# Ren-Okubo/diffusion_model

Hardware: AMD Instinct MI355X
Metric: atoms*denoise-steps/sec, 64-atom SiO2 T=1000 (higher is better)
Workload: dtype bf16; 1 GPU; 64-atom SiO2 cells x 256 graphs/GPU, 4-layer EGNN (H=36, W=1024, m=256), T=1000 reverse steps, fully connected (E=1032192/GPU); global_batch=256, parallelism=replicas x1 (no data-path collective)

## Files before the change

diffusion_model_amd/csrc/edge_tile.h:

```cpp
#pragma once
#include "kernels.h"

namespace egnn {
namespace tile128 {

constexpr int kR = 128;
static_assert(kR == kTileRows, "plan_forward (host_logic.cpp) plans 128-edge tiles");
constexpr int kSegFast = 8;
constexpr int kTileThreads = 512;
constexpr int kChunkK = 64;
constexpr int kRowPad = kR + 1;
constexpr size_t kChunkBytes = (size_t)8 * kRowPad * 16;
constexpr size_t kStageBytes = (size_t)8 * 32 * 72 * 2;
constexpr size_t kOffDst = 0;
constexpr size_t kOffSrc = kOffDst + kR * 4;
constexpr size_t kOffD2 = kOffSrc + kR * 4;
constexpr size_t kOffDiff = kOffD2 + kR * 4;
constexpr size_t kOffVal = kOffDiff + 3 * kR * 4;
constexpr size_t kOffPart = kOffVal + kR * 4;
constexpr size_t kOffSegRow = kOffPart + 8 * kR * 4;
constexpr size_t kOffSegNode = kOffSegRow + kR * 4;
constexpr size_t kOffSegRs = kOffSegNode + kR * 4;
constexpr size_t kOffSegRe = kOffSegRs + kR * 4;
constexpr size_t kOffSegMode = kOffSegRe + kR * 4;
constexpr size_t kOffMisc = kOffSegMode + kR * 4;
constexpr size_t kOffGseg = kOffMisc + 64;
constexpr size_t kOffLoop = kOffGseg + kSegFast * kR * 4;

#define TILE_LDS_RD(dst, base, off) asm volatile("ds_read_b128 %0, %1 offset:%2" : "=v"(dst) : "v"(base), "n"(off))
#define TILE_LDS_WAIT(n) asm volatile("s_waitcnt lgkmcnt(" #n ")" ::: "memory")

struct Lds {
  int *dst, *src, *seg_of_row, *seg_node, *seg_rs, *seg_re, *seg_mode, *misc;
  float *d2, *diff, *val, *part, *gseg;
  __device__ __forceinline__ explicit Lds(char* smem)
      : dst(reinterpret_cast<int*>(smem + kOffDst)), src(reinterpret_cast<int*>(smem + kOffSrc)),
        seg_of_row(reinterpret_cast<int*>(smem + kOffSegRow)), seg_node(reinterpret_cast<int*>(smem + kOffSegNode)),
        seg_rs(reinterpret_cast<int*>(smem + kOffSegRs)), seg_re(reinterpret_cast<int*>(smem + kOffSegRe)),
        seg_mode(reinterpret_cast<int*>(smem + kOffSegMode)), misc(reinterpret_cast<int*>(smem + kOffMisc)),
        d2(reinterpret_cast<float*>(smem + kOffD2)), diff(reinterpret_cast<float*>(smem + kOffDiff)),
        val(reinterpret_cast<float*>(smem + kOffVal)), part(reinterpret_cast<float*>(smem + kOffPart)),
        gseg(reinterpret_cast<float*>(smem + kOffGseg)) {}
};

__device__ __forceinline__ void prologue_rows(const EdgeParams& p, const Lds& L, int e0, int nvalid, const float* wd, int KP,
                                              float* s_wd, int tid) {
  if (tid < kR) {
    int d = 0, s = 0;
    float dx = 0.f, dy = 0.f, dz = 0.f;
    if (tid < nvalid) {
      d = p.edge_dst[e0 + tid];
      s = p.edge_src[e0 + tid];
      dx = p.x[3 * d] - p.x[3 * s];
      dy = p.x[3 * d + 1] - p.x[3 * s + 1];
      dz = p.x[3 * d + 2] - p.x[3 * s + 2];
    }
    L.dst[tid] = d;
    L.src[tid] = s;
    L.diff[tid] = dx; L.diff[kR + tid] = dy; L.diff[2 * kR + tid] = dz;
    const float nrm = sqrtf(dx * dx + dy * dy + dz * dz);
    L.d2[tid] = nrm * nrm;
  }
  for (int i = tid; i < KP; i += 512) s_wd[i] = wd[i];
  __syncthreads();
}

__device__ __forceinline__ int segment_mode(const EdgeParams& p, const Lds& L, int e0, int seg) {
  const int n = L.seg_node[seg];
  const bool first = (e0 + L.seg_rs[seg]) == p.row_ptr[n];
  const bool last = (e0 + L.seg_re[seg] + 1) == p.row_ptr[n + 1];
  return (first && last) ? 2 : (first ? 1 : 0);
}

template <bool WITH_MODES = true>
__device__ __forceinline__ int prologue_segments(const EdgeParams& p, const Lds& L, int e0, int nvalid, int tid, int lane, int wave) {
  bool is_start = false, is_end = false;
  unsigned long long starts = 0;
  if (tid < kR) {
    const bool valid = tid < nvalid;
    const int d = L.dst[tid];
    is_start = valid && (tid == 0 || L.dst[tid - 1] != d);
    is_end = valid && (tid == nvalid - 1 || L.dst[tid + 1] != d);
    starts = __ballot(is_start);
    if (lane == 0) L.misc[1 + wave] = __popcll(starts);
  }
  __syncthreads();
  if (tid < kR) {
    const int seg = (wave == 1 ? L.misc[1] : 0) + __popcll(starts & ((2ull << lane) - 1ull)) - 1;
    L.seg_of_row[tid] = tid < nvalid ? seg : -1;
    if (is_start) { L.seg_node[seg] = L.dst[tid]; L.seg_rs[seg] = tid; }
    if (is_end) L.seg_re[seg] = tid;
    if (tid == 0) L.misc[0] = L.misc[1] + L.misc[2];
  }
  __syncthreads();
  const int S = L.misc[0];
  if constexpr (WITH_MODES) {
    if (tid < S) L.seg_mode[tid] = segment_mode(p, L, e0, tid);
  }
  return S;
}

__device__ __forceinline__ int prologue(const EdgeParams& p, const Lds& L, int e0, int nvalid, const float* wd, int KP,
                                        float* s_wd, int tid, int lane, int wave) {
  prologue_rows(p, L, e0, nvalid, wd, KP, s_wd, tid);
  return prologue_segments(p, L, e0, nvalid, tid, lane, wave);
}

template <int ESZ>
struct BuildRows {
  int brow, kg;
  unsigned vdst0, vsrc0, vdst1, vsrc1, offP, offQ;
  float d2r0, d2r1;
  rsrc_t tab;
  __device__ __forceinline__ unsigned row_off(const EdgeParams& p, int node) const {
    return (unsigned)node * (unsigned)p.TC * (unsigned)ESZ + (unsigned)kg * (8u * ESZ);
  }
  __device__ __forceinline__ BuildRows(const EdgeParams& p, const Lds& L, int tid, bool is_m, unsigned table_bytes, int d0, int s0,
                                       int d1, int s1)
      : brow(tid >> 3), kg(tid & 7), vdst0(row_off(p, d0)), vsrc0(row_off(p, s0)), vdst1(row_off(p, d1)), vsrc1(row_off(p, s1)),
        offP((is_m ? 2u * p.WxP : 0u) * ESZ), offQ((is_m ? 2u * p.WxP + p.WmP : (unsigned)p.WxP) * ESZ), d2r0(L.d2[brow]),
        d2r1(L.d2[brow + 64]), tab(make_rsrc(p.table, table_bytes)) {}
  __device__ __forceinline__ BuildRows(const EdgeParams& p, const Lds& L, int tid, bool is_m, unsigned table_bytes)
      : brow(tid >> 3), kg(tid & 7), vdst0(row_off(p, L.dst[brow])), vsrc0(row_off(p, L.src[brow])),
        vdst1(row_off(p, L.dst[brow + 64])), vsrc1(row_off(p, L.src[brow + 64])), offP((is_m ? 2u * p.WxP : 0u) * ESZ),
        offQ((is_m ? 2u * p.WxP + p.WmP : (unsigned)p.WxP) * ESZ), d2r0(L.d2[brow]), d2r1(L.d2[brow + 64]),
        tab(make_rsrc(p.table, table_bytes)) {}
};

template <class MPhase, class VFinish, class VLoad>
__device__ __forceinline__ void phase_opposed_k_loop(int NC, int wave, MPhase&& mphase, VFinish&& vfinish, VLoad&& vload) {
  if (wave < 4) {
    vload(1);
    for (int i = 0; i < NC - 1; ++i) {
      mphase(i, false);
      vfinish(i + 1);
      vload(i + 2);
      __syncthreads();
    }
    mphase(NC - 1, true);
    __syncthreads();
  } else {
    vload(1);
    for (int i = 0; i < NC - 1; ++i) {
      vfinish(i + 1);
      vload(i + 2);
      __builtin_amdgcn_sched_barrier(0);
      mphase(i, false);
      __syncthreads();
    }
    mphase(NC - 1, true);
    __syncthreads();
  }
}

template <int CB>
__device__ __forceinline__ void stage_store_rows(const f32x16 (&acc)[4][CB], char* stage, __bf16* out, size_t ld, int nvalid,
                                                 int lane, int wave) {
  static_assert(CB == 1 || CB == 2, "store_block_bf16 takes one or two 32-column blocks");
  __bf16* stg = reinterpret_cast<__bf16*>(stage) + (size_t)wave * 32 * 72;
#pragma unroll
  for (int rb = 0; rb < 4; ++rb) {
    f32x16 blk[2];
    blk[0] = acc[rb][0];
    blk[1] = acc[rb][CB - 1];
    store_block_bf16(blk, CB, stg, out + (size_t)(32 * rb) * ld, ld, nvalid - 32 * rb, lane);
  }
}

__device__ __forceinline__ void coordinate_segment_sums(const EdgeParams& p, const Lds& L, int S, int tile, int half, int tid,
                                                        int lane, int wave) {
  float* aggx = p.agg_x + (size_t)half * p.agg_x_stride;
  float* partx = p.part_x + (size_t)half * p.part_x_stride;
  if (S <= kSegFast) {
    if (wave < S) {
      const int seg = wave;
      float a0 = 0.f, a1 = 0.f, a2 = 0.f, a3 = 0.f;
#pragma unroll
      for (int u = 0; u < 2; ++u) {
        const int row = lane + 64 * u;
        if (L.seg_of_row[row] == seg) {
          const float sv = L.val[row];
          const float dx = L.diff[row], dy = L.diff[kR + row], dz = L.diff[2 * kR + row];
          a0 += dx * sv; a1 += dy * sv; a2 += dz * sv;
          a3 += dx * dx + dy * dy + dz * dz;
        }
      }
#pragma unroll
      for (int m = 32; m >= 1; m >>= 1) { a0 += __shfl_xor(a0, m); a1 += __shfl_xor(a1, m); a2 += __shfl_xor(a2, m); a3 += __shfl_xor(a3, m); }
      if (lane < 4) {
        const int mode = L.seg_mode[seg];
        float* dstp = mode == 2 ? aggx + (size_t)L.seg_node[seg] * 4 : partx + ((size_t)tile * 2 + mode) * 4;
        dstp[lane] = lane == 0 ? a0 : (lane == 1 ? a1 : (lane == 2 ? a2 : a3));
      }
    }
  } else {
    for (int t = tid; t < 4 * S; t += 512) {
      const int seg = t >> 2, d = t & 3, mode = L.seg_mode[seg];
      float sum = 0.f;
      if (d < 3) {
        for (int rr = L.seg_rs[seg]; rr <= L.seg_re[seg]; ++rr) sum += L.diff[d * kR + rr] * L.val[rr];
      } else {
        for (int rr = L.seg_rs[seg]; rr <= L.seg_re[seg]; ++rr) {
          const float dx = L.diff[rr], dy = L.diff[kR + rr], dz = L.diff[2 * kR + rr];
          sum += dx * dx + dy * dy + dz * dz;
        }
      }
      float* dstp = mode == 2 ? aggx + (size_t)L.seg_node[seg] * 4 : partx + ((size_t)tile * 2 + mode) * 4;
      dstp[d] = sum;
    }
  }
}



template <int CB, bool PRE_SCALED = false, bool STORE_SHARE = false>
__device__ __forceinline__ void x_head(const EdgeParams& p, const Lds& L, const f32x16 (&acc)[4][CB], int colblk0, int half,
                                       int tid, int lane, int wave, const float acc_scale = kNegLog2e, int e0 = 0,
                                       int nvalid = 0) {
  const int r = lane & 31;
  float part[64];
#pragma unroll
  for (int q = 0; q < 64; ++q) part[q] = 0.f;
#pragma unroll
  for (int cb = 0; cb < CB; ++cb) {
    const int n = 32 * (colblk0 + cb) + r;
    const float bb = p.b2x[n], w = p.w3x[n];
#pragma unroll
    for (int rb = 0; rb < 4; ++rb)
#pragma unroll
      for (int i = 0; i < 16; ++i)
        part[rb * 16 + i] = fmaf(w, silu_s(PRE_SCALED ? acc[rb][cb][i] : fmaf(acc[rb][cb][i], acc_scale, bb)), part[rb * 16 + i]);
  }
  {
    float lo[32], hi[32];
#pragma unroll
    for (int q = 0; q < 32; ++q) { lo[q] = part[q]; hi[q] = part[32 + q]; }
    const float t0 = butterfly32(lo, lane), t1 = butterfly32(hi, lane);
    const int row = 32 * (r >> 4) + acc_row(r & 15, lane);
    L.part[wave * kR + row] = t0;
    L.part[wave * kR + 64 + row] = t1;
  }
  __syncthreads();
  if (tid < kR) {
    float v = half == 0 ? p.scal[0] : 0.f;
#pragma unroll
    for (int w = 0; w < 8; ++w) v += L.part[w * kR + tid];
    L.val[tid] = v;
    if constexpr (STORE_SHARE) { if (tid < nvalid) p.s_half_out[(size_t)half * p.E + e0 + tid] = v; }
  }
  __syncthreads();
}

template <bool PRE_SCALED = false>
__device__ __forceinline__ void message_epilogue(const EdgeParams& p, const Lds& L, const f32x16 (&acc)[4][1], int S, int tile,
                                                 int tid, int lane, int wave, const float acc_scale = kNegLog2e,
                                                 const int colblk = -1) {
  const int r = lane & 31, hh = lane >> 5;
  const int ncol = 32 * (colblk < 0 ? wave : colblk) + r;
  float mval[64];
  {
    const float bb = p.b2m[ncol], wa = p.wa[ncol];
    float lo[32], hi[32];
#pragma unroll
    for (int rb = 0; rb < 4; ++rb)
#pragma unroll
      for (int i = 0; i < 16; ++i) {
        const float m = silu_s(PRE_SCALED ? acc[rb][0][i] : fmaf(acc[rb][0][i], acc_scale, bb));
        mval[rb * 16 + i] = m;
        if (rb < 2) lo[rb * 16 + i] = wa * m; else hi[(rb - 2) * 16 + i] = wa * m;
      }
    const float t0 = butterfly32(lo, lane), t1 = butterfly32(hi, lane);
    const int row = 32 * (r >> 4) + acc_row(r & 15, lane);
    L.part[wave * kR + row] = t0;
    L.part[wave * kR + 64 + row] = t1;
  }
  __syncthreads();
  if (tid < kR) {
    float g = p.scal[1];
#pragma unroll
    for (int w = 0; w < 8; ++w) g += L.part[w * kR + tid];
    L.val[tid] = sigmoid_f(g) * kNegInvLog2e;
  }
  __syncthreads();
  for (int base = 0; base < S; base += kSegFast) {
    const int ns = min(kSegFast, S - base);
    if (base > 0) __syncthreads();
    for (int t = tid; t < ns * kR; t += 512) {
      const int seg = base + (t >> 7), row = t & 127;
      L.gseg[t] = (L.seg_of_row[row] == seg) ? L.val[row] : 0.f;
    }
    __syncthreads();
    for (int sg = 0; sg < ns; ++sg) {
      const int seg = base + sg;
      const float* gw = L.gseg + sg * kR + 4 * hh;
      float v = 0.f;
#pragma unroll
      for (int rb = 0; rb < 4; ++rb)
#pragma unroll
        for (int i = 0; i < 16; ++i) v = fmaf(mval[rb * 16 + i], gw[32 * rb + (i & 3) + 8 * (i >> 2)], v);
      v += __shfl_xor(v, 32);
      if (hh == 0) {
        const int mode = L.seg_mode[seg];
        float* dstp = mode == 2 ? p.agg_m + (size_t)L.seg_node[seg] * p.MP : p.part_m + ((size_t)tile * 2 + mode) * p.MP;
        dstp[ncol] = v;
      }
    }
  }
}

__device__ __forceinline__ void butterfly16(float (&v)[32], int lane, float& out0, float& out1) {
#pragma unroll
  for (int q = 0; q < 16; ++q) {
    const float ta = v[q] + dpp_mov<0x128>(v[q]);
    const float tb = v[q + 16] + dpp_mov<0x128>(v[q + 16]);
    v[q] = dpp_sel<0xC>(ta, tb);
  }
#pragma unroll
  for (int q = 0; q < 8; ++q) {
    const float ta = v[q] + dpp_mov<0x141>(v[q]);
    const float tb = v[q + 8] + dpp_mov<0x141>(v[q + 8]);
    v[q] = dpp_sel<0xA>(ta, tb);
  }
  const bool b2 = (lane & 2) != 0, b1 = (lane & 1) != 0;
#pragma unroll
  for (int q = 0; q < 4; ++q) {
    const float ta = v[q] + dpp_mov<0x4E>(v[q]);
    const float tb = v[q + 4] + dpp_mov<0x4E>(v[q + 4]);
    v[q] = b2 ? tb : ta;
  }
#pragma unroll
  for (int q = 0; q < 2; ++q) {
    const float ta = v[q] + dpp_mov<0xB1>(v[q]);
    const float tb = v[q + 2] + dpp_mov<0xB1>(v[q + 2]);
    v[q] = b1 ? tb : ta;
  }
  out0 = v[0];
  out1 = v[1];
}

}
}
```

diffusion_model_amd/csrc/edge_x_m16.hip:

```cpp
#include <cstdlib>

#include "diag.h"
#include "edge_tile.h"

namespace egnn {

namespace {

#ifdef EGNN_EXP_WGSTAMP
__device__ unsigned long long g_xwg_stamps[20000][12];
#define WG_STAMP(k) DIAG_WG_STAMP(g_xwg_stamps, 20000, k)
#define WG_STAMP_HW() DIAG_WG_STAMP_HW(g_xwg_stamps, 20000, 5)
#else
#define WG_STAMP(k)
#define WG_STAMP_HW()
#endif

using namespace tile128;
constexpr size_t kA1 = (size_t)8 * kR * 16;
__host__ __device__ constexpr size_t x16_smem_bytes(int KP) { return kOffLoop + 2 * kA1 + (size_t)KP * 4; }
static_assert(x16_smem_bytes(256) == 48192 && x16_smem_bytes(512) == 49216 && x16_smem_bytes(1024) == 51264,
              "LDS allocation of the 16x16x32 coordinate kernels");
constexpr int kKept = 6;
__host__ __device__ constexpr size_t x16_persist_smem_bytes(int KP) { return x16_smem_bytes(KP) + (KP == 1024 ? kKept * kA1 : 0); }
static_assert(x16_persist_smem_bytes(512) == 49216 && x16_persist_smem_bytes(1024) == 149568 && x16_persist_smem_bytes(1024) <= 160 * 1024,
              "LDS allocation of the persistent 16x16x32 coordinate kernel");

typedef __attribute__((ext_vector_type(4))) float f32x4v;

template <bool SAVE, typename V8 = bf16x8, bool PERSIST = false>
__global__ __launch_bounds__(kTileThreads, 2) void edge_x_m16_kernel(const EdgeParams p) {
  static_assert(!(SAVE && OpTraits<V8>::f16), "the training forward keeps bf16 activations");
  static_assert(!(SAVE && PERSIST), "the persistent form is the inference kernel");
  if constexpr (OpTraits<V8>::f16) f16_saturate_mode();
  extern __shared__ __attribute__((aligned(16))) char smem[];
  const Lds L(smem);
  char* s_a1 = smem + kOffLoop;
  float* s_wd = reinterpret_cast<float*>(s_a1 + 2 * kA1);

  const int tid = threadIdx.x, lane = tid & 63;
  const int wave = __builtin_amdgcn_readfirstlane(tid >> 6);
  const int r15 = lane & 15, q4 = lane >> 4;
  const int KP = p.WxP;
  const int nsplit = p.WxP / 512;
  const int NC = KP / kChunkK, KS = KP / 32;
  const rsrc_t rs_tab = make_rsrc(p.table, diag::drop_table_loads(p.dbg) ? 0u : (unsigned)((size_t)p.N * p.TC * 2));
  const rsrc_t rs_w = make_rsrc(p.w2x, diag::drop_weight_loads(p.dbg) ? 0u : (unsigned)((size_t)p.WxP * KP * 2));
  const unsigned offP = 0u, offQ = (unsigned)p.WxP * 2u;
  const unsigned lane16 = lane * 16u;
  const int ntiles = (p.E + kR - 1) / kR;
  const rsrc_t rs_tab0 = make_rsrc(p.table, 0u);
  UnitH uc0, uc1;
  V8 bq[2][4];
  int pf_d0, pf_s0, pf_d1, pf_s1, pf_d, pf_s, pf_r0, pf_r1;
  float pf_x[6];
  auto prefetch_indices = [&](const int t, const int tq) {
    const int ne0 = t * kR, nnv = min(kR, p.E - ne0), br = tq >> 3;
    const bool r0 = br < nnv, r1 = br + 64 < nnv, rt = tq < nnv && tq < kR;
    pf_d0 = r0 ? p.edge_dst[ne0 + br] : 0; pf_s0 = r0 ? p.edge_src[ne0 + br] : 0;
    pf_d1 = r1 ? p.edge_dst[ne0 + br + 64] : 0; pf_s1 = r1 ? p.edge_src[ne0 + br + 64] : 0;
    pf_d = rt ? p.edge_dst[ne0 + tq] : 0; pf_s = rt ? p.edge_src[ne0 + tq] : 0;
  };
  auto prefetch_data = [&](const int h, const rsrc_t tab, const int tq) {
    const unsigned k16 = (unsigned)(tq & 7) * 16u, l16 = (unsigned)(tq & 63) * 16u;
#pragma unroll
    for (int k = 0; k < 3; ++k) { pf_x[k] = p.x[3 * pf_d + k]; pf_x[3 + k] = p.x[3 * pf_s + k]; }
    pf_r0 = p.row_ptr[pf_d]; pf_r1 = p.row_ptr[pf_d + 1];
    unith_load(uc0, tab, (unsigned)pf_d0 * (unsigned)p.TC * 2u + k16, (unsigned)pf_s0 * (unsigned)p.TC * 2u + k16, offP, offQ);
    unith_load(uc1, tab, (unsigned)pf_d1 * (unsigned)p.TC * 2u + k16, (unsigned)pf_s1 * (unsigned)p.TC * 2u + k16, offP, offQ);
    const unsigned nw0 = (unsigned)(h * 32 + wave * 4) * KS * 1024u;
#pragma unroll
    for (int s = 0; s < 2; ++s)
#pragma unroll
      for (int cb = 0; cb < 4; ++cb) bq[s][cb] = ldbuf_v8<V8>(rs_w, l16, nw0 + ((unsigned)cb * KS + s) * 1024u);
  };
  XUnit cur{0, 0, false, true};
  int kstep = 0;
  if constexpr (PERSIST) {
    cur = x_walk(blockIdx.x, gridDim.x, ntiles, nsplit, 0);
    if (!cur.valid) return;
    for (int i = tid; i < KP; i += kTileThreads) s_wd[i] = p.wdx[i];
    prefetch_indices(cur.tile, tid);
    prefetch_data(cur.share, rs_tab, tid);
  }
  do {
  const int j = PERSIST ? 0 : xcd_tile(blockIdx.x, gridDim.x);
  const int tile = PERSIST ? cur.tile : j / nsplit, half = PERSIST ? cur.share : j - tile * nsplit;
  const bool kept = PERSIST && cur.kept, skip = kept && half == 1;
  const unsigned kept_off = 2u * (unsigned)kA1 + (unsigned)KP * 4u;
  auto chunk_off = [&](const int c) -> unsigned {
    return (kept && c < kKept) ? kept_off + (unsigned)c * (unsigned)kA1 : (unsigned)(c & 1) * (unsigned)kA1;
  };
  const int e0 = tile * kR;
  const int nvalid = min(kR, p.E - e0);

  DIAG_STAMP_SETUP(p.stamps + (size_t)wave * 32 * 4);
  DIAG_STAMP(30, 0);
  WG_STAMP(0);
  int tid_p = tid;
  if constexpr (PERSIST) asm volatile("" : "+v"(tid_p));
  const int lane_p = tid_p & 63;
  if constexpr (!PERSIST) {
    prologue_rows(p, L, e0, nvalid, p.wdx, KP, s_wd, tid);
  } else if (!skip) {
    const int tid = tid_p;
    if (tid < kR) {
      const float dx = pf_x[0] - pf_x[3], dy = pf_x[1] - pf_x[4], dz = pf_x[2] - pf_x[5];
      L.dst[tid] = pf_d;
      L.src[tid] = pf_s;
      L.diff[tid] = dx; L.diff[kR + tid] = dy; L.diff[2 * kR + tid] = dz;
      const float nrm = sqrtf(dx * dx + dy * dy + dz * dz);
      L.d2[tid] = nrm * nrm;
      reinterpret_cast<int*>(L.gseg)[tid] = pf_r0;
      reinterpret_cast<int*>(L.gseg)[kR + tid] = pf_r1;
    }
    __syncthreads();
  }
  DIAG_STAMP(30, 1);
  WG_STAMP(1);

  const BuildRows<2> b(p, L, tid, false, diag::drop_table_loads(p.dbg) ? 0u : (unsigned)((size_t)p.N * p.TC * 2),
                       PERSIST ? pf_d0 : L.dst[tid >> 3], PERSIST ? pf_s0 : L.src[tid >> 3], PERSIST ? pf_d1 : L.dst[(tid >> 3) + 64],
                       PERSIST ? pf_s1 : L.src[(tid >> 3) + 64]);
  char* slot0 = s_a1 + (size_t)b.kg * (kR * 16) + (size_t)(b.brow ^ b.kg) * 16;
  char* slot1 = slot0 + 64 * 16;
  const unsigned lds0 = (unsigned)(size_t)(__attribute__((address_space(3))) char*)s_a1;
  const unsigned abase0 = lds0 + (unsigned)q4 * (kR * 16) + (unsigned)(r15 ^ q4) * 16u;
  const unsigned abase1 = lds0 + (unsigned)(4 + q4) * (kR * 16) + (unsigned)(r15 ^ (4 + q4)) * 16u;
  const int cb0 = half * 32 + wave * 4;
  const unsigned w0 = (unsigned)cb0 * KS * 1024u;

  f32x4v acc[8][4];
#pragma unroll
  for (int rb = 0; rb < 8; ++rb)
#pragma unroll
    for (int cb = 0; cb < 4; ++cb)
#pragma unroll
      for (int i = 0; i < 4; ++i) acc[rb][cb][i] = 0.f;

  const rsrc_t rs_s1 = make_rsrc(SAVE ? p.s1_out : nullptr, SAVE ? (unsigned)((size_t)p.E * KP * 2) : 0u);
  const unsigned vs1_0 = (unsigned)(e0 + b.brow) * (unsigned)KP * 2u + (unsigned)b.kg * 16u, vs1_1 = vs1_0 + 64u * (unsigned)KP * 2u;
  auto s1_store = [&](const V8 o0, const V8 o1, const int c) {
    if (half != 0) return;
    if constexpr (diag::kNoS1) return;
    const unsigned soff = __builtin_amdgcn_readfirstlane((unsigned)c * kChunkK * 2u);
    __builtin_amdgcn_raw_buffer_store_b128(__builtin_bit_cast(u32x4, o0), rs_s1, vs1_0, soff, 0);
    __builtin_amdgcn_raw_buffer_store_b128(__builtin_bit_cast(u32x4, o1), rs_s1, vs1_1, soff, 0);
  };
  if constexpr (!PERSIST) {
    unith_load(uc0, b.tab, b.vdst0, b.vsrc0, b.offP, b.offQ);
    unith_load(uc1, b.tab, b.vdst1, b.vsrc1, b.offP, b.offQ);
#pragma unroll
    for (int s = 0; s < 2; ++s)
#pragma unroll
      for (int cb = 0; cb < 4; ++cb) bq[s][cb] = ldbuf_v8<V8>(rs_w, lane16, w0 + ((unsigned)cb * KS + s) * 1024u);
  }
  int S;
  if (!skip) S = prologue_segments<false>(p, L, e0, nvalid, tid_p, lane_p, wave);
  else S = L.misc[0];
  if constexpr (PERSIST) {
    if (!skip && tid_p < S) {
      const int* rp = reinterpret_cast<const int*>(L.gseg);
      const int r0 = L.seg_rs[tid_p];
      const bool first = (e0 + r0) == rp[r0], last = (e0 + L.seg_re[tid_p] + 1) == rp[kR + r0];
      L.seg_mode[tid_p] = (first && last) ? 2 : (first ? 1 : 0);
    }
  }
  if (!skip) {
    const V8 o0 = unith_finish<V8>(uc0, s_wd + b.kg * 8, b.d2r0, slot0 + chunk_off(0));
    const V8 o1 = unith_finish<V8>(uc1, s_wd + b.kg * 8, b.d2r1, slot1 + chunk_off(0));
    if constexpr (SAVE) s1_store(o0, o1, 0);
  }
  __syncthreads();

  auto mphase = [&](const int c, const bool last) {
    const unsigned boff = chunk_off(c);
    const unsigned ab0 = abase0 + boff, ab1 = abase1 + boff;
    V8 a[3];
    TILE_LDS_RD(a[0], ab0, 0); TILE_LDS_RD(a[1], ab0, 256); TILE_LDS_RD(a[2], ab0, 512);
#pragma unroll
    for (int s = 0; s < 2; ++s) {
#pragma unroll
      for (int rb = 0; rb < 8; ++rb) {
        const int u = 8 * s + rb;
        if (u <= 13) TILE_LDS_WAIT(2);
        else if (u == 14) TILE_LDS_WAIT(1);
        else TILE_LDS_WAIT(0);
        asm volatile("" : "+v"(a[u % 3]));
#pragma unroll
        for (int cb = 0; cb < 4; ++cb)
          acc[rb][cb] = mfma16(a[u % 3], bq[s][cb], acc[rb][cb]);
#ifdef XM16_PIN
        __builtin_amdgcn_sched_barrier(0);
#endif
        if (u == 0) TILE_LDS_RD(a[0], ab0, 768); if (u == 1) TILE_LDS_RD(a[1], ab0, 1024); if (u == 2) TILE_LDS_RD(a[2], ab0, 1280);
        if (u == 3) TILE_LDS_RD(a[0], ab0, 1536); if (u == 4) TILE_LDS_RD(a[1], ab0, 1792); if (u == 5) TILE_LDS_RD(a[2], ab1, 0);
        if (u == 6) TILE_LDS_RD(a[0], ab1, 256); if (u == 7) TILE_LDS_RD(a[1], ab1, 512); if (u == 8) TILE_LDS_RD(a[2], ab1, 768);
        if (u == 9) TILE_LDS_RD(a[0], ab1, 1024); if (u == 10) TILE_LDS_RD(a[1], ab1, 1280); if (u == 11) TILE_LDS_RD(a[2], ab1, 1536);
        if (u == 12) TILE_LDS_RD(a[0], ab1, 1792);
      }
      if (!last) {
        const unsigned ksn = (unsigned)((c + 1) * 2 + s) * 1024u;
#pragma unroll
        for (int cb = 0; cb < 4; ++cb) bq[s][cb] = ldbuf_v8<V8>(rs_w, lane16, w0 + (unsigned)cb * KS * 1024u + ksn);
      }
    }
  };
  UnitH ua0, ua1;
  auto vload = [&](const int cq) {
    const int c = cq < NC ? cq : NC - 1;
    const unsigned kb = (unsigned)c * kChunkK * 2u;
    unith_load(ua0, b.tab, b.vdst0, b.vsrc0, b.offP + kb, b.offQ + kb);
    unith_load(ua1, b.tab, b.vdst1, b.vsrc1, b.offP + kb, b.offQ + kb);
  };
  auto vfinish = [&](const int c) {
    const size_t nbuf = chunk_off(c);
    __builtin_amdgcn_s_setprio(3);
    const V8 o0 = unith_finish<V8>(ua0, s_wd + c * kChunkK + b.kg * 8, b.d2r0, slot0 + nbuf);
    const V8 o1 = unith_finish<V8>(ua1, s_wd + c * kChunkK + b.kg * 8, b.d2r1, slot1 + nbuf);
    __builtin_amdgcn_s_setprio(0);
    if constexpr (SAVE) s1_store(o0, o1, c);
  };
  DIAG_STAMP(30, 2);
  WG_STAMP(2);
  DIAG_RSTAMP(31, 1);
  const int istart = skip ? kKept - 1 : 0;
  if (wave < 4) {
    const int my_mode = (!PERSIST && tid_p < S) ? segment_mode(p, L, e0, tid_p) : 0;
    if constexpr (PERSIST) for (int i = 0; i < istart; ++i) mphase(i, false);
    vload(istart + 1);
    for (int i = istart; i < NC - 1; ++i) {
      mphase(i, false);
      if (!PERSIST && i == 0 && tid_p < S) L.seg_mode[tid_p] = my_mode;
      vfinish(i + 1);
      vload(i + 2);
      __syncthreads();
    }
  } else {
    if constexpr (PERSIST) for (int i = 0; i < istart - 1; ++i) mphase(i, false);
    vload(istart + 1);
    if constexpr (PERSIST) { if (skip) mphase(istart - 1, false); }
    for (int i = istart; i < NC - 1; ++i) {
      vfinish(i + 1);
      vload(i + 2);
      __builtin_amdgcn_sched_barrier(0);
      mphase(i, false);
      __syncthreads();
    }
  }
  mphase(NC - 1, true);
  __syncthreads();
  DIAG_STAMP(30, 3);
  WG_STAMP(3);
  DIAG_RSTAMP(31, 2);

  int tid_e = tid;
  if constexpr (PERSIST) asm volatile("" : "+v"(tid_e));
  const int lane_e = tid_e & 63, r15_e = lane_e & 15, q4_e = lane_e >> 4;
  XUnit nxt = cur;
  bool more = false;
  if constexpr (PERSIST) {
    const XUnit n2 = x_walk(blockIdx.x, gridDim.x, ntiles, nsplit, kstep + 1);
    more = n2.valid;
    if (more) nxt = n2;
    prefetch_indices(nxt.tile, tid_e);
  }
  float part[32];
#pragma unroll
  for (int v = 0; v < 32; ++v) part[v] = 0.f;
  if constexpr (SAVE && !diag::kNoStage) {
#pragma unroll
    for (int cb = 0; cb < 4; ++cb) {
      const float bb = p.b2x[16 * (cb0 + cb) + r15_e];
#pragma unroll
      for (int rb = 0; rb < 8; ++rb)
#pragma unroll
        for (int i = 0; i < 4; ++i) acc[rb][cb][i] = fmaf(acc[rb][cb][i], kNegLog2e, bb);
    }
    typedef __attribute__((ext_vector_type(2))) unsigned u32x2s;
    char* tile = s_a1 + (size_t)wave * (64 * 32);
    const unsigned tile_lds = (unsigned)(size_t)(__attribute__((address_space(3))) char*)tile;
    const int g16 = lane_e >> 4, j16 = lane_e & 15;
    const unsigned rd_addr = tile_lds + (unsigned)((8 * g16 + (j16 >> 2)) * 32 + (j16 & 3) * 8);
    __bf16* tout = static_cast<__bf16*>(p.g_a2_out) + (size_t)e0 * p.WxP + 16 * cb0;
#pragma unroll
    for (int rb = 0; rb < 8; ++rb) {
#pragma unroll
      for (int cb = 0; cb < 4; ++cb) {
        u32x2s w;
        asm("v_cvt_pk_bf16_f32 %0, %1, %2" : "=v"(w.x) : "v"(acc[rb][cb][0]), "v"(acc[rb][cb][1]));
        asm("v_cvt_pk_bf16_f32 %0, %1, %2" : "=v"(w.y) : "v"(acc[rb][cb][2]), "v"(acc[rb][cb][3]));
        *reinterpret_cast<u32x2s*>(tile + (16 * cb + r15_e) * 32 + q4_e * 8) = w;
      }
      __builtin_amdgcn_wave_barrier();
      u32x2s t[2][2];
      asm volatile("s_waitcnt lgkmcnt(0)\n\t"
                   "ds_read_b64_tr_b16 %0, %4 offset:0\n\t"
                   "ds_read_b64_tr_b16 %1, %4 offset:128\n\t"
                   "ds_read_b64_tr_b16 %2, %4 offset:1024\n\t"
                   "ds_read_b64_tr_b16 %3, %4 offset:1152\n\t"
                   "s_waitcnt lgkmcnt(0)"
                   : "=&v"(t[0][0]), "=&v"(t[0][1]), "=&v"(t[1][0]), "=&v"(t[1][1]) : "v"(rd_addr) : "memory");
      if (16 * rb + j16 < nvalid - (diag::kNoT2 ? 1000 : 0)) {
#pragma unroll
        for (int k = 0; k < 2; ++k) {
          const u32x4 o = {t[k][0].x, t[k][0].y, t[k][1].x, t[k][1].y};
          *reinterpret_cast<u32x4*>(tout + (size_t)(16 * rb + j16) * p.WxP + 32 * k + 8 * g16) = o;
        }
      }
      __builtin_amdgcn_wave_barrier();
    }
  }
  typedef __attribute__((ext_vector_type(2))) float f32x2;
#pragma unroll
  for (int cb = 0; cb < 4; ++cb) {
    const int n = 16 * (cb0 + cb) + r15_e;
    const float bb = p.b2x[n], w = p.w3x[n];
    constexpr float kAcc = kNegLog2e / OpTraits<V8>::wscale;
    const f32x2 bb2 = {bb, bb}, w2 = {w, w}, k2 = {kAcc, kAcc}, one2 = {1.0f, 1.0f};
#pragma unroll
    for (int rb = 0; rb < 8; ++rb)
#pragma unroll
      for (int i = 0; i < 4; i += 2) {
        const f32x2 a2 = {acc[rb][cb][i], acc[rb][cb][i + 1]};
        const f32x2 t = SAVE ? a2 : __builtin_elementwise_fma(a2, k2, bb2);
        const f32x2 e = {__builtin_amdgcn_exp2f(t.x), __builtin_amdgcn_exp2f(t.y)};
        const f32x2 d = e + one2;
        const f32x2 rr = {__builtin_amdgcn_rcpf(d.x), __builtin_amdgcn_rcpf(d.y)};
        const f32x2 sv = t * rr;
        f32x2 pp = {part[rb * 4 + i], part[rb * 4 + i + 1]};
        pp = __builtin_elementwise_fma(w2, sv, pp);
        part[rb * 4 + i] = pp.x;
        part[rb * 4 + i + 1] = pp.y;
      }
  }
  WG_STAMP(6);
  if constexpr (PERSIST) prefetch_data(nxt.share, more && nxt.kept && nxt.share == 1 ? rs_tab0 : rs_tab, tid_e);
  {
    float t0, t1;
    butterfly16(part, lane_e, t0, t1);
    const int row = 16 * (r15_e >> 1) + 4 * q4_e + 2 * (r15_e & 1);
    L.part[wave * kR + row] = t0;
    L.part[wave * kR + row + 1] = t1;
  }
  __syncthreads();
  WG_STAMP(7);
  if (tid_e < kR) {
    float v = half == 0 ? p.scal[0] : 0.f;
#pragma unroll
    for (int w = 0; w < 8; ++w) v += L.part[w * kR + tid_e];
    L.val[tid_e] = v;
    if constexpr (SAVE) { if (tid_e < nvalid && p.s_half_out) p.s_half_out[(size_t)half * p.E + e0 + tid_e] = v; }
  }
  __syncthreads();
  WG_STAMP(8);
  coordinate_segment_sums(p, L, S, tile, half, tid_e, lane_e, wave);
  DIAG_STAMP(31, 0);
  WG_STAMP(4);
  WG_STAMP_HW();
  if constexpr (!PERSIST) break;
  if (!more) break;
  cur = nxt;
  ++kstep;
  __syncthreads();
  } while (true);
}

}

int init_edge_x_m16_attributes() {
  EGNN_HIP(hipFuncSetAttribute(reinterpret_cast<const void*>(&edge_x_m16_kernel<false>), hipFuncAttributeMaxDynamicSharedMemorySize,
                               160 * 1024));
  EGNN_HIP(hipFuncSetAttribute(reinterpret_cast<const void*>(&edge_x_m16_kernel<true>), hipFuncAttributeMaxDynamicSharedMemorySize,
                               160 * 1024));
  EGNN_HIP(hipFuncSetAttribute(reinterpret_cast<const void*>(&edge_x_m16_kernel<false, f16x8>), hipFuncAttributeMaxDynamicSharedMemorySize,
                               160 * 1024));
  EGNN_HIP(hipFuncSetAttribute(reinterpret_cast<const void*>(&edge_x_m16_kernel<false, bf16x8, true>), hipFuncAttributeMaxDynamicSharedMemorySize,
                               160 * 1024));
  EGNN_HIP(hipFuncSetAttribute(reinterpret_cast<const void*>(&edge_x_m16_kernel<false, f16x8, true>), hipFuncAttributeMaxDynamicSharedMemorySize,
                               160 * 1024));
  return EGNN_OK;
}

bool edge_x_m16_supported(const EdgeParams& p) {
  return (p.WxP == 512 || p.WxP == 1024) && p.w2x16 != nullptr && x16_persist_smem_bytes(p.WxP) <= 160 * 1024 &&
         (size_t)p.N * p.TC * 2 < ((size_t)1 << 32);
}

int launch_edge_x_m16(const EdgeParams& p, hipStream_t st, bool f16, XForm form, int grid) {
  const int units = (p.E + kR - 1) / kR * (p.WxP / 512);
  const size_t sm = x16_smem_bytes(p.WxP), smp = x16_persist_smem_bytes(p.WxP);
  EdgeParams q = p;
  q.w2x = p.w2x16;
  switch (form) {
    case XForm::kSave:
      if (f16) { set_error("edge_x_m16: the training forward runs on bf16 operands"); return EGNN_EINVAL; }
      hipLaunchKernelGGL(edge_x_m16_kernel<true>, dim3(units), dim3(kTileThreads), sm, st, q);
      break;
    case XForm::kPersistent:
      if (f16) hipLaunchKernelGGL((edge_x_m16_kernel<false, f16x8, true>), dim3(grid), dim3(kTileThreads), smp, st, q);
      else hipLaunchKernelGGL((edge_x_m16_kernel<false, bf16x8, true>), dim3(grid), dim3(kTileThreads), smp, st, q);
      break;
    case XForm::kPerUnit:
      if (f16) hipLaunchKernelGGL((edge_x_m16_kernel<false, f16x8>), dim3(units), dim3(kTileThreads), sm, st, q);
      else hipLaunchKernelGGL(edge_x_m16_kernel<false>, dim3(units), dim3(kTileThreads), sm, st, q);
      break;
  }
  EGNN_HIP(hipGetLastError());
  return EGNN_OK;
}

}

#ifdef EGNN_EXP_WGSTAMP
extern "C" int egnn_debug_xwg_stamps(unsigned long long* host_out) {
  return hipMemcpyFromSymbol(host_out, HIP_SYMBOL(egnn::g_xwg_stamps), sizeof(unsigned long long) * 20000 * 12) == hipSuccess ? 0 : -1;
}
#endif
```

diffusion_model_amd/csrc/x_walk.h:

```cpp
#pragma once

#if defined(__HIPCC__)
#define EGNN_XWALK_HD __host__ __device__ __forceinline__
#else
#define EGNN_XWALK_HD inline
#endif

namespace egnn {

EGNN_XWALK_HD int xcd_tile(int b, int nwg) {
  const int xcd = b & 7, q = nwg >> 3, r = nwg & 7;
  return (xcd < r ? xcd * (q + 1) : r * (q + 1) + (xcd - r) * q) + (b >> 3);
}

struct XUnit {
  int tile, share;
  bool kept, valid;
};

EGNN_XWALK_HD XUnit x_walk(int b, int G, int T, int nshare, int k) {
  const int S = T / G, R = T - S * G;
  XUnit u;
  if (k < nshare * S) {
    const int sweep = k / nshare;
    u.tile = sweep * G + xcd_tile(b, G);
    u.share = k - sweep * nshare;
    u.kept = nshare == 2;
    u.valid = true;
  } else {
    const int v0 = (k - nshare * S) * G;
    const int left = nshare * R - v0;
    const int n = left < G ? left : G;
    u.valid = b < n;
    const int v = u.valid ? v0 + xcd_tile(b, n) : 0;
    u.tile = S * G + v / nshare;
    u.share = v % nshare;
    u.kept = false;
  }
  return u;
}

}
```

Baseline: 1.716 million atoms*denoise-steps/s.

## Keep seven LDS chunks across coordinate-kernel shares and rotate chunk order

Result: no change. 1.722 million atoms*denoise-steps/s, median of 6 (+0.4%).

```diff
diff --git a/diffusion_model_amd/csrc/edge_tile.h b/diffusion_model_amd/csrc/edge_tile.h
--- a/diffusion_model_amd/csrc/edge_tile.h
+++ b/diffusion_model_amd/csrc/edge_tile.h
@@ -26,6 +26,9 @@
 constexpr size_t kOffMisc = kOffSegMode + kR * 4;
 constexpr size_t kOffGseg = kOffMisc + 64;
 constexpr size_t kOffLoop = kOffGseg + kSegFast * kR * 4;
+constexpr size_t kOffRowPtrX = kOffGseg;
+constexpr size_t kOffLoopX = kOffRowPtrX + 2 * kR * 4;
+static_assert(kOffLoop == 14400 && kOffLoopX == 11328 && kOffLoopX % 16 == 0, "LDS carve of the per-tile arrays");
 
 #define TILE_LDS_RD(dst, base, off) asm volatile("ds_read_b128 %0, %1 offset:%2" : "=v"(dst) : "v"(base), "n"(off))
 #define TILE_LDS_WAIT(n) asm volatile("s_waitcnt lgkmcnt(" #n ")" ::: "memory")
diff --git a/diffusion_model_amd/csrc/edge_x_m16.hip b/diffusion_model_amd/csrc/edge_x_m16.hip
--- a/diffusion_model_amd/csrc/edge_x_m16.hip
+++ b/diffusion_model_amd/csrc/edge_x_m16.hip
@@ -18,12 +18,13 @@
 
 using namespace tile128;
 constexpr size_t kA1 = (size_t)8 * kR * 16;
-__host__ __device__ constexpr size_t x16_smem_bytes(int KP) { return kOffLoop + 2 * kA1 + (size_t)KP * 4; }
-static_assert(x16_smem_bytes(256) == 48192 && x16_smem_bytes(512) == 49216 && x16_smem_bytes(1024) == 51264,
+__host__ __device__ constexpr size_t x16_smem_bytes(int KP) { return kOffLoopX + 2 * kA1 + (size_t)KP * 4; }
+static_assert(x16_smem_bytes(256) == 45120 && x16_smem_bytes(512) == 46144 && x16_smem_bytes(1024) == 48192,
               "LDS allocation of the 16x16x32 coordinate kernels");
-constexpr int kKept = 6;
+constexpr int kKept = kXKept;
+static_assert(x_kept(1024 / kChunkK) == kKept, "x_chunk (x_walk.h) orders the chunks for this many kept buffers");
 __host__ __device__ constexpr size_t x16_persist_smem_bytes(int KP) { return x16_smem_bytes(KP) + (KP == 1024 ? kKept * kA1 : 0); }
-static_assert(x16_persist_smem_bytes(512) == 49216 && x16_persist_smem_bytes(1024) == 149568 && x16_persist_smem_bytes(1024) <= 160 * 1024,
+static_assert(x16_persist_smem_bytes(512) == 46144 && x16_persist_smem_bytes(1024) == 162880 && x16_persist_smem_bytes(1024) <= 160 * 1024,
               "LDS allocation of the persistent 16x16x32 coordinate kernel");
 
 typedef __attribute__((ext_vector_type(4))) float f32x4v;
@@ -35,8 +36,9 @@
   if constexpr (OpTraits<V8>::f16) f16_saturate_mode();
   extern __shared__ __attribute__((aligned(16))) char smem[];
   const Lds L(smem);
-  char* s_a1 = smem + kOffLoop;
+  char* s_a1 = smem + kOffLoopX;
   float* s_wd = reinterpret_cast<float*>(s_a1 + 2 * kA1);
+  int* s_rp = reinterpret_cast<int*>(smem + kOffRowPtrX);
 
   const int tid = threadIdx.x, lane = tid & 63;
   const int wave = __builtin_amdgcn_readfirstlane(tid >> 6);
@@ -62,7 +64,8 @@
     pf_d = rt ? p.edge_dst[ne0 + tq] : 0; pf_s = rt ? p.edge_src[ne0 + tq] : 0;
   };
   auto prefetch_data = [&](const int h, const rsrc_t tab, const int tq) {
-    const unsigned k16 = (unsigned)(tq & 7) * 16u, l16 = (unsigned)(tq & 63) * 16u;
+    const unsigned c0 = (unsigned)x_chunk(nsplit, h, 0, NC);
+    const unsigned k16 = c0 * kChunkK * 2u + (unsigned)(tq & 7) * 16u, l16 = (unsigned)(tq & 63) * 16u;
 #pragma unroll
     for (int k = 0; k < 3; ++k) { pf_x[k] = p.x[3 * pf_d + k]; pf_x[3 + k] = p.x[3 * pf_s + k]; }
     pf_r0 = p.row_ptr[pf_d]; pf_r1 = p.row_ptr[pf_d + 1];
@@ -72,7 +75,7 @@
 #pragma unroll
     for (int s = 0; s < 2; ++s)
 #pragma unroll
-      for (int cb = 0; cb < 4; ++cb) bq[s][cb] = ldbuf_v8<V8>(rs_w, l16, nw0 + ((unsigned)cb * KS + s) * 1024u);
+      for (int cb = 0; cb < 4; ++cb) bq[s][cb] = ldbuf_v8<V8>(rs_w, l16, nw0 + ((unsigned)cb * KS + 2u * c0 + s) * 1024u);
   };
   XUnit cur{0, 0, false, true};
   int kstep = 0;
@@ -89,8 +92,11 @@
   const bool kept = PERSIST && cur.kept, skip = kept && half == 1;
   const unsigned kept_off = 2u * (unsigned)kA1 + (unsigned)KP * 4u;
   auto chunk_off = [&](const int c) -> unsigned {
-    return (kept && c < kKept) ? kept_off + (unsigned)c * (unsigned)kA1 : (unsigned)(c & 1) * (unsigned)kA1;
-  };
+    const int buf = x_buffer(kept, c, NC);
+    return buf >= 2 ? kept_off + (unsigned)(buf - 2) * (unsigned)kA1 : (unsigned)buf * (unsigned)kA1;
+  };
+  auto ord = [&](const int i) -> int { return x_chunk(nsplit, half, i, NC); };
+  const int c0 = ord(0);
   const int e0 = tile * kR;
   const int nvalid = min(kR, p.E - e0);
 
@@ -111,8 +117,8 @@
       L.diff[tid] = dx; L.diff[kR + tid] = dy; L.diff[2 * kR + tid] = dz;
       const float nrm = sqrtf(dx * dx + dy * dy + dz * dz);
       L.d2[tid] = nrm * nrm;
-      reinterpret_cast<int*>(L.gseg)[tid] = pf_r0;
-      reinterpret_cast<int*>(L.gseg)[kR + tid] = pf_r1;
+      s_rp[tid] = pf_r0;
+      s_rp[kR + tid] = pf_r1;
     }
     __syncthreads();
   }
@@ -148,32 +154,32 @@
     __builtin_amdgcn_raw_buffer_store_b128(__builtin_bit_cast(u32x4, o1), rs_s1, vs1_1, soff, 0);
   };
   if constexpr (!PERSIST) {
-    unith_load(uc0, b.tab, b.vdst0, b.vsrc0, b.offP, b.offQ);
-    unith_load(uc1, b.tab, b.vdst1, b.vsrc1, b.offP, b.offQ);
+    const unsigned kb0 = (unsigned)c0 * kChunkK * 2u;
+    unith_load(uc0, b.tab, b.vdst0, b.vsrc0, b.offP + kb0, b.offQ + kb0);
+    unith_load(uc1, b.tab, b.vdst1, b.vsrc1, b.offP + kb0, b.offQ + kb0);
 #pragma unroll
     for (int s = 0; s < 2; ++s)
 #pragma unroll
-      for (int cb = 0; cb < 4; ++cb) bq[s][cb] = ldbuf_v8<V8>(rs_w, lane16, w0 + ((unsigned)cb * KS + s) * 1024u);
+      for (int cb = 0; cb < 4; ++cb) bq[s][cb] = ldbuf_v8<V8>(rs_w, lane16, w0 + ((unsigned)cb * KS + 2u * (unsigned)c0 + s) * 1024u);
   }
   int S;
   if (!skip) S = prologue_segments<false>(p, L, e0, nvalid, tid_p, lane_p, wave);
   else S = L.misc[0];
   if constexpr (PERSIST) {
     if (!skip && tid_p < S) {
-      const int* rp = reinterpret_cast<const int*>(L.gseg);
       const int r0 = L.seg_rs[tid_p];
-      const bool first = (e0 + r0) == rp[r0], last = (e0 + L.seg_re[tid_p] + 1) == rp[kR + r0];
+      const bool first = (e0 + r0) == s_rp[r0], last = (e0 + L.seg_re[tid_p] + 1) == s_rp[kR + r0];
       L.seg_mode[tid_p] = (first && last) ? 2 : (first ? 1 : 0);
     }
   }
   if (!skip) {
-    const V8 o0 = unith_finish<V8>(uc0, s_wd + b.kg * 8, b.d2r0, slot0 + chunk_off(0));
-    const V8 o1 = unith_finish<V8>(uc1, s_wd + b.kg * 8, b.d2r1, slot1 + chunk_off(0));
-    if constexpr (SAVE) s1_store(o0, o1, 0);
+    const V8 o0 = unith_finish<V8>(uc0, s_wd + c0 * kChunkK + b.kg * 8, b.d2r0, slot0 + chunk_off(c0));
+    const V8 o1 = unith_finish<V8>(uc1, s_wd + c0 * kChunkK + b.kg * 8, b.d2r1, slot1 + chunk_off(c0));
+    if constexpr (SAVE) s1_store(o0, o1, c0);
   }
   __syncthreads();
 
-  auto mphase = [&](const int c, const bool last) {
+  auto mphase = [&](const int c, const int cn, const bool last) {
     const unsigned boff = chunk_off(c);
     const unsigned ab0 = abase0 + boff, ab1 = abase1 + boff;
     V8 a[3];
@@ -200,15 +206,15 @@
         if (u == 12) TILE_LDS_RD(a[0], ab1, 1792);
       }
       if (!last) {
-        const unsigned ksn = (unsigned)((c + 1) * 2 + s) * 1024u;
+        const unsigned ksn = (unsigned)(cn * 2 + s) * 1024u;
 #pragma unroll
         for (int cb = 0; cb < 4; ++cb) bq[s][cb] = ldbuf_v8<V8>(rs_w, lane16, w0 + (unsigned)cb * KS * 1024u + ksn);
       }
     }
   };
   UnitH ua0, ua1;
-  auto vload = [&](const int cq) {
-    const int c = cq < NC ? cq : NC - 1;
+  auto vload = [&](const int iq) {
+    const int c = ord(iq < NC ? iq : NC - 1);
     const unsigned kb = (unsigned)c * kChunkK * 2u;
     unith_load(ua0, b.tab, b.vdst0, b.vsrc0, b.offP + kb, b.offQ + kb);
     unith_load(ua1, b.tab, b.vdst1, b.vsrc1, b.offP + kb, b.offQ + kb);
@@ -224,31 +230,32 @@
   DIAG_STAMP(30, 2);
   WG_STAMP(2);
   DIAG_RSTAMP(31, 1);
-  const int istart = skip ? kKept - 1 : 0;
+  const int istart = skip ? kKept + 1 : 0;
   if (wave < 4) {
     const int my_mode = (!PERSIST && tid_p < S) ? segment_mode(p, L, e0, tid_p) : 0;
-    if constexpr (PERSIST) for (int i = 0; i < istart; ++i) mphase(i, false);
+    if constexpr (PERSIST) for (int i = 0; i < istart; ++i) mphase(ord(i), ord(i + 1), false);
     vload(istart + 1);
+    if constexpr (PERSIST) { if (skip) __syncthreads(); }
     for (int i = istart; i < NC - 1; ++i) {
-      mphase(i, false);
+      mphase(ord(i), ord(i + 1), false);
       if (!PERSIST && i == 0 && tid_p < S) L.seg_mode[tid_p] = my_mode;
-      vfinish(i + 1);
+      vfinish(ord(i + 1));
       vload(i + 2);
       __syncthreads();
     }
   } else {
-    if constexpr (PERSIST) for (int i = 0; i < istart - 1; ++i) mphase(i, false);
+    if constexpr (PERSIST) for (int i = 0; i < istart - 1; ++i) mphase(ord(i), ord(i + 1), false);
     vload(istart + 1);
-    if constexpr (PERSIST) { if (skip) mphase(istart - 1, false); }
+    if constexpr (PERSIST) { if (skip) { mphase(ord(istart - 1), ord(istart), false); __syncthreads(); } }
     for (int i = istart; i < NC - 1; ++i) {
-      vfinish(i + 1);
+      vfinish(ord(i + 1));
       vload(i + 2);
       __builtin_amdgcn_sched_barrier(0);
-      mphase(i, false);
+      mphase(ord(i), ord(i + 1), false);
       __syncthreads();
     }
   }
-  mphase(NC - 1, true);
+  mphase(ord(NC - 1), 0, true);
   __syncthreads();
   DIAG_STAMP(30, 3);
   WG_STAMP(3);
diff --git a/diffusion_model_amd/csrc/x_walk.h b/diffusion_model_amd/csrc/x_walk.h
--- a/diffusion_model_amd/csrc/x_walk.h
+++ b/diffusion_model_amd/csrc/x_walk.h
@@ -40,4 +40,13 @@
   return u;
 }
 
+constexpr int kXKept = 7;
+EGNN_XWALK_HD constexpr int x_kept(int NC) { return NC - 2 < kXKept ? NC - 2 : kXKept; }
+EGNN_XWALK_HD constexpr int x_buffer(bool kept, int c, int NC) { return (kept && c < x_kept(NC)) ? 2 + c : (c & 1); }
+EGNN_XWALK_HD constexpr int x_chunk(int nshare, int share, int i, int NC) {
+  const int first = (nshare == 2 && share == 0) ? x_kept(NC) + 2 : 0;
+  const int c = i + first;
+  return c < NC ? c : c - NC;
 }
+
+}
```
